# CapAI/ship-sim-gym

Hardware: AMD Instinct MI355X
Metric: env steps/sec (batched ShipEnv) (higher is better)
Workload: dtype f64

## Files before the change

### ship_sim_gym_amd/csrc/shipsim_kernels.hip

```cpp
#include <hip/hip_runtime.h>

#include <cfloat>
#include <cstdint>
#include <type_traits>

#include "shipsim.h"
#include "shipsim_internal.h"

namespace ssg {

__device__ __forceinline__ double *lds_base()
{
    extern __shared__ double s_lds[];
    return s_lds;
}

__device__ __forceinline__ double dmin(double a, double b) { return __builtin_fmin(a, b); }
__device__ __forceinline__ double dmax(double a, double b) { return __builtin_fmax(a, b); }

__device__ __forceinline__ double obs_fma(double a, double b, double c)
{
#ifndef SSG_NO_LIDAR_FMA
    return __builtin_fma(a, b, c);
#else
    return a * b + c;
#endif
}

__device__ __forceinline__ double readlane_f64(double v, int src_lane)
{
    const int lo = __builtin_amdgcn_readlane(__double2loint(v), src_lane);
    const int hi = __builtin_amdgcn_readlane(__double2hiint(v), src_lane);
    return __hiloint2double(hi, lo);
}

__device__ __forceinline__ void set_f64(double &d, double v) { asm volatile("v_mov_b64 %0, %1" : "+v"(d) : "v"(v)); }
__device__ __forceinline__ void set_f64_uniform(double &d, double s) { asm volatile("v_mov_b64 %0, %1" : "+v"(d) : "s"(s)); }
__device__ __forceinline__ void set_f64_zero(double &d) { asm volatile("v_mov_b64 %0, 0" : "+v"(d)); }
__device__ __forceinline__ void set_f64_one(double &d) { asm volatile("v_mov_b64 %0, 1.0" : "+v"(d)); }
__device__ __forceinline__ void set_f64_minus_one(double &d) { asm volatile("v_mov_b64 %0, -1.0" : "+v"(d)); }
template <class T> __device__ __forceinline__ void set_b32(T &d, T v) { static_assert(sizeof(T) == 4, "one register"); asm volatile("v_mov_b32 %0, %1" : "+v"(d) : "v"(v)); }
__device__ __forceinline__ void set_b32_uniform(int &d, int s) { asm volatile("v_mov_b32 %0, %1" : "+v"(d) : "s"(s)); }
template <class T> __device__ __forceinline__ void set_b32_zero(T &d) { static_assert(sizeof(T) == 4, "one register"); asm volatile("v_mov_b32 %0, 0" : "+v"(d)); }

__device__ __attribute__((noinline)) double2 sincos_call(double a)
{
    double2 o;
    sincos_body(a, &o.x, &o.y);
    return o;
}

__device__ __forceinline__ double ld_f64(const double *p, bool fresh)
{
    if (fresh)
        return __longlong_as_double((long long)__hip_atomic_load(reinterpret_cast<const unsigned long long *>(p),
                                                                  __ATOMIC_RELAXED, __HIP_MEMORY_SCOPE_AGENT));
    return *p;
}
__device__ __forceinline__ int ld_i32(const int32_t *p, bool fresh)
{
    if (fresh) return __hip_atomic_load(p, __ATOMIC_RELAXED, __HIP_MEMORY_SCOPE_AGENT);
    return *p;
}
__device__ __forceinline__ unsigned ld_u8(const uint8_t *p, bool fresh)
{
    if (fresh) return __hip_atomic_load(p, __ATOMIC_RELAXED, __HIP_MEMORY_SCOPE_AGENT);
    return *p;
}

template <bool LDS_BANK>
__device__ __forceinline__ double bank_at(const DevCfg &c, int i)
{
    if constexpr (LDS_BANK) return lds_base()[i];
    else return c.bank[i];
}
template <bool LDS_BANK>
__device__ __forceinline__ double2 bank_at2(const DevCfg &c, int i)
{
    if constexpr (LDS_BANK) { double2 r; r.x = lds_base()[i]; r.y = lds_base()[i + 1]; return r; }
    else {
        typedef double double2_a8 __attribute__((ext_vector_type(2), aligned(8)));
        const double2_a8 v = *reinterpret_cast<const double2_a8 *>(c.bank + i);
        double2 r; r.x = v.x; r.y = v.y; return r;
    }
}

template <int THREADS>
__device__ __forceinline__ void stage_bank_lds(const double *__restrict__ bank, int bytes, double &tail_v, int &tail_o)
{
    const int wave = threadIdx.x >> 6, lane = threadIdx.x & 63;
    constexpr int NW = THREADS / 64;
    const int nchunk = bytes >> 10;
    const char *g = reinterpret_cast<const char *>(bank);
    char *l = reinterpret_cast<char *>(lds_base());
    for (int ch = wave; ch < nchunk; ch += NW) {
        __builtin_amdgcn_global_load_lds((const __attribute__((address_space(1))) void *)(g + (size_t)ch * 1024 + lane * 16),
                                         (__attribute__((address_space(3))) void *)(l + ch * 1024), 16, 0, 0);
    }
    const int tail0 = nchunk << 10;
    const int o = tail0 + (int)threadIdx.x * 8;
    tail_o = (o < bytes) ? o : -1;
    tail_v = 0.0;
    if (o < bytes) tail_v = *reinterpret_cast<const double *>(g + o);
    static_assert(THREADS * 8 >= 1024, "tail copy needs one thread per 8 bytes of a 1 KiB chunk");
}

template <bool LDS_BANK, bool DYN>
__device__ __forceinline__ double goal_at(const DevCfg &c, int goff, int g, int comp)
{
    if constexpr (DYN) return c.dyn_f64[(size_t)(DC_GOALS + DC_GOAL_COLS * g + comp) * (size_t)c.n_pad + goff];
    else return bank_at<LDS_BANK>(c, goff + 2 * g + comp);
}

template <bool LDS_BANK, bool DYN>
__device__ __forceinline__ void nearest_goal(const DevCfg &c, int goff, unsigned gm, double x, double y, double &gx,
                                             double &gy, const double *hG = nullptr , int ld = 0)
{
    gx = -1.0;
    gy = -1.0;
    double best = INFINITY;
    int gi = -1;
    if constexpr (!LDS_BANK && !DYN) {
#pragma unroll
        for (int g = 0; g < SSG_MAX_GOALS; ++g) {
            if (g >= c.n_goals) break;
            const double px = hG[(2 * g) * ld], py = hG[(2 * g + 1) * ld];
// ... 36 lines not shown
}

__device__ __forceinline__ int next_map(const DevCfg &c, int map_id, int env)
{
    if (c.map_ring > 0) {
        const int base = env * c.map_ring;
        const int nxt = map_id + 1;
        return (nxt - base >= c.map_ring) ? base : nxt;
    }
    const int nxt = map_id + 1;
    return (nxt >= c.n_maps) ? 0 : nxt;
}

__device__ __forceinline__ void beam_end(double cx, double cy, double ca, double sa, double cphi, double sphi, double dist,
                                         double &ex, double &ey)
{
    const double ux = obs_fma(ca, cphi, -(sa * sphi)), uy = obs_fma(sa, cphi, ca * sphi);
    ex = obs_fma(dist, ux, cx);
    ey = obs_fma(dist, uy, cy);
}

__host__ __device__ __forceinline__ constexpr int nb_lo(int nb) { return (nb + 1) / 2; }
constexpr int kBeamTabBytes = 2 * SSG_MAX_BEAMS * 8;
constexpr int kShipTabBytes = 6 * 8 * 8;
constexpr int kTrafficTabBytes = SSG_N_TRAFFIC * 4 * 8 * 8;
constexpr int kPoseDoubles = 7;
constexpr int kGoalScratchBytes = 64 * SSG_MAX_GOALS * 2 + 64 * 4;
constexpr int kTrafficScratchBytes = 64 * SSG_N_TRAFFIC * 2 + 64 * 4;
__host__ __device__ __forceinline__ constexpr int lds_fixed_bytes(int epw, bool dyn)
{
    return kBeamTabBytes + kShipTabBytes + (dyn ? kTrafficTabBytes : 0) + kPoseDoubles * epw * 8 + (dyn ? 8 : 6) * epw * 4 + 4 * (epw / 64) * 4 +
           (epw / 64) * (kGoalScratchBytes + (dyn ? kTrafficScratchBytes : 0));
}
__host__ __device__ __forceinline__ constexpr int lds_res_bytes(int nb) { return nb * 64 * 8; }
__host__ __device__ __forceinline__ constexpr int lds_queue_bytes(int nb0) { return (2 * nb0 * 64 + 64) * 2; }
__host__ __device__ __forceinline__ constexpr int lds_tile_bytes(int nb)
{
    return 2 * lds_res_bytes(nb) + 2 * lds_queue_bytes(nb_lo(nb));
}

constexpr int kHdrLidar = 10, kHdrGoals = 2 * SSG_MAX_GOALS;
static_assert(SSG_MAP_OFF_COUNTS == 0 && SSG_MAP_OFF_AABB == 2 && SSG_MAP_OFF_GOALS == kHdrLidar && SSG_MAP_OFF_SPAWN_GOAL == kHdrLidar + kHdrGoals,
              "the record's head: counts, boxes, goals, spawn goal");
#ifndef SSG_SIX_ROLE_MAX_EPW
#define SSG_SIX_ROLE_MAX_EPW 128
#endif
__host__ __device__ __forceinline__ constexpr int tile_roles(int epw, bool dyn) { return (epw <= SSG_SIX_ROLE_MAX_EPW && !dyn) ? 6 : 4; }
__host__ __device__ __forceinline__ constexpr int lds_hdr_bytes(int epw, bool lds_bank, bool dyn) { return lds_bank ? 0 : ((tile_roles(epw, dyn) - 2) * kHdrLidar + kHdrGoals) * epw * 8; }

constexpr unsigned long long kLidarMiss = ~0ull;

template <bool LDS_BANK> struct PlaneChunk { static constexpr int n = LDS_BANK ? 4 : 8; };

template <bool EXACT>
__device__ __forceinline__ double seg_mad(double a, double b, double c) { return EXACT ? a * b + c : obs_fma(a, b, c); }

template <bool LDS_BANK, bool EXACT>
__device__ __forceinline__ void lidar_pass(const DevCfg &c, const int n_items, const unsigned short *queue,
                                           unsigned long long *res , const double *beamtab,
                                           const double cx, const double cy, const double ca, const double sa,
                                           const int rec_off, const int lane, const double *hLt = nullptr , const int ld = 0)
{
    for (int base = 0; base < n_items; base += 64) {
        const int idx = base + lane;
        const bool act = idx < n_items;
        const unsigned code = queue[act ? idx : 0];
        const int src = code & 63, bi = (code >> 6) & (SSG_MAX_BEAMS - 1), s = (code >> 10) & 1;
        const double wcx = __shfl(cx, src), wcy = __shfl(cy, src), wca = __shfl(ca, src), wsa = __shfl(sa, src);
        const int woff = __shfl(rec_off, src);
        double ex, ey;
        beam_end(wcx, wcy, wca, wsa, beamtab[bi], beamtab[SSG_MAX_BEAMS + bi], c.lidar_dist, ex, ey);
        int cnt;
        if constexpr (LDS_BANK) cnt = (int)bank_at<LDS_BANK>(c, woff + SSG_MAP_OFF_COUNTS + s);
        else cnt = (int)hLt[s * ld + src];
        const int pb = woff + SSG_MAP_OFF_PLANES + s * (SSG_MAX_HULL * SSG_PLANE_DOUBLES);
        bool outside = false;
        bool out_sure = false, maybe = false;
        constexpr double kSignEps = 1e-9;
        bool ok = false;
        double ptx = ex, pty = ey;
        double bd = -1.0, bden = 1.0, t_hit = 0.0;
        int bj = 0;
        constexpr int kPlaneChunk = PlaneChunk<LDS_BANK>::n;
        for (int j0 = 0; __any(act & (j0 < cnt)); j0 += kPlaneChunk) {
            double pv0x[kPlaneChunk], pv0y[kPlaneChunk], pnx[kPlaneChunk], pny[kPlaneChunk], pv0n[kPlaneChunk];
            double pdtmin[kPlaneChunk], pdtmax[kPlaneChunk];
#pragma unroll
            for (int u = 0; u < kPlaneChunk; ++u) {
                const int j = j0 + u;
                const int q = pb + SSG_PLANE_DOUBLES * ((j < SSG_MAX_HULL) ? j : 0);
                const bool want = LDS_BANK || (act & (j < cnt));
                pv0x[u] = pv0y[u] = pnx[u] = pny[u] = pv0n[u] = 0.0;
                if (EXACT && want) { const double2 vv = bank_at2<LDS_BANK>(c, q + 0); pv0x[u] = vv.x; pv0y[u] = vv.y; }
                if (want) { const double2 nn = bank_at2<LDS_BANK>(c, q + 2); pnx[u] = nn.x; pny[u] = nn.y; }
                if (want) pv0n[u] = bank_at<LDS_BANK>(c, q + 4);
                if (EXACT) {
                    const int jp = (j == 0) ? cnt - 1 : j - 1;
                    const int qp = pb + SSG_PLANE_DOUBLES * ((jp >= 0 && jp < SSG_MAX_HULL) ? jp : 0);
                    const double ux = bank_at<LDS_BANK>(c, qp + 0), uy = bank_at<LDS_BANK>(c, qp + 1);
                    pdtmin[u] = seg_mad<EXACT>(pnx[u], uy, -(pny[u] * ux));
                    pdtmax[u] = seg_mad<EXACT>(pnx[u], pv0y[u], -(pny[u] * pv0x[u]));
                }
            }
#pragma unroll
            for (int u = 0; u < kPlaneChunk; ++u) {
                const int j = j0 + u;
                const bool valid = act & (j < cnt);
                const double nx = pnx[u], ny = pny[u], v0n = pv0n[u];
                const double an = seg_mad<EXACT>(wcx, nx, wcy * ny);
                const double d = an - v0n;
                if (EXACT) {
                    outside = outside | (valid & ((nx * (wcx - pv0x[u]) + ny * (wcy - pv0y[u])) > 0.0));
                } else {
                    out_sure = out_sure | (valid & (d > kSignEps));
                    maybe = maybe | (valid & !(d < -kSignEps));
                }
                const bool front = valid & !(d < 0.0);
                const double bn = seg_mad<EXACT>(ex, nx, ey * ny);
                const double den = dmax(an - bn, DBL_MIN);
                if (EXACT) {
                    const double t = d / den;
                    const double omt = 1.0 - t;
                    const double qx = seg_mad<EXACT>(ex, t, wcx * omt), qy = seg_mad<EXACT>(ey, t, wcy * omt);
                    const double dtv = seg_mad<EXACT>(nx, qy, -(ny * qx));
                    const bool acc = front & !((t < 0.0) | (1.0 < t)) & (pdtmin[u] <= dtv) & (dtv <= pdtmax[u]);
                    ok = ok | acc;
                    ptx = acc ? qx : ptx;
                    pty = acc ? qy : pty;
                } else {
                    const bool better = front & (d <= den) & (d * bden >= bd * den);
#ifdef SSG_NO_MASKED_BEST
                    bd = better ? d : bd;
                    bden = better ? den : bden;
                    bj = better ? j : bj;
#else
                    if (better) { set_f64(bd, d); set_f64(bden, den); set_b32_uniform(bj, j); }
#endif
                }
            }
        }
        if (!EXACT) {
            outside = out_sure;
            const bool need_exact = act & !out_sure & maybe;
            if (__any(need_exact)) {
                bool o = false;
                for (int j = 0; __any(need_exact & (j < cnt)); ++j) {
                    const int qq = pb + SSG_PLANE_DOUBLES * ((j < SSG_MAX_HULL) ? j : 0);
                    const double v0x = bank_at<LDS_BANK>(c, qq + 0), v0y = bank_at<LDS_BANK>(c, qq + 1);
                    const double nx = bank_at<LDS_BANK>(c, qq + 2), ny = bank_at<LDS_BANK>(c, qq + 3);
                    o = o | ((j < cnt) & ((nx * (wcx - v0x) + ny * (wcy - v0y)) > 0.0));
                }
                outside = need_exact ? o : outside;
            }
            const int q = pb + SSG_PLANE_DOUBLES * bj;
            const int jp = (bj == 0) ? cnt - 1 : bj - 1;
            const int qp = pb + SSG_PLANE_DOUBLES * ((jp >= 0 && jp < SSG_MAX_HULL) ? jp : 0);
            double2 nn = bank_at2<LDS_BANK>(c, q + 2), vj = bank_at2<LDS_BANK>(c, q + 0), vp = bank_at2<LDS_BANK>(c, qp + 0);
            if constexpr (!LDS_BANK) asm volatile("" : "+v"(nn.x), "+v"(nn.y), "+v"(vj.x), "+v"(vj.y), "+v"(vp.x), "+v"(vp.y));
            const double nx = nn.x, ny = nn.y;
            const double dtmin = obs_fma(nx, vp.y, -(ny * vp.x));
            const double dtmax = obs_fma(nx, vj.y, -(ny * vj.x));
            const double t = bd / bden;
            const double omt = 1.0 - t;
            ptx = obs_fma(ex, t, wcx * omt);
            pty = obs_fma(ey, t, wcy * omt);
            const double dtv = obs_fma(nx, pty, -(ny * ptx));
            ok = (bd >= 0.0) & (dtmin <= dtv) & (dtv <= dtmax);
            t_hit = t;
        }
        const bool hit = act & (ok | !outside);
        double dist;
        if constexpr (EXACT) {
            const double px = outside ? ptx : ex, py = outside ? pty : ey;
            const double dx = px - wcx, dy = py - wcy;
            dist = sqrt(dx * dx + dy * dy);
        } else {
            dist = outside ? t_hit * c.lidar_dist : c.lidar_dist;
        }
        if (hit) {
            const unsigned long long key = ((unsigned long long)s << 63) | (unsigned long long)__double_as_longlong(dist);
            atomicMin(&res[bi * 64 + src], key);
        }
#ifdef SSG_LIDAR_COUNT
        if (c.dbg) {
            const unsigned long long ma = __ballot(act), mh = __ballot(hit), mo = __ballot(act & !outside);
            if (lane == 0) { atomicAdd(c.dbg + 65536 + 0, (unsigned long long)__popcll(ma)); atomicAdd(c.dbg + 65536 + 1, (unsigned long long)__popcll(mh));
                             atomicAdd(c.dbg + 65536 + 2, 1ull); atomicAdd(c.dbg + 65536 + 3, (unsigned long long)__popcll(mo)); }
        }
#endif
    }
}

template <class T>
__device__ __forceinline__ void st_out(T *p, T v)
{
#ifdef SSG_WT
    __hip_atomic_store(p, v, __ATOMIC_RELAXED, __HIP_MEMORY_SCOPE_AGENT);
#else
    *p = v;
#endif
}

#ifdef SSG_STAMPS
#define SSG_STAMP(k)                                                                              \
    do {                                                                                          \
        __builtin_amdgcn_sched_barrier(0);                                                        \
        unsigned long long t_;                                                                    \
        asm volatile("s_memtime %0\n\ts_waitcnt lgkmcnt(0)" : "=s"(t_)::"memory");               \
        __builtin_amdgcn_sched_barrier(0);                                                        \
        stamp_[k] = t_;                                                                           \
    } while (0)
#define SSG_STAMP_FLUSH(n)                                                                        \
    do {                                                                                          \
        if (c.dbg && lane == 0) {                                                                 \
            unsigned long long *d_ = c.dbg + 16 * (size_t)(blockIdx.x * (NR * EPW / 64) + (threadIdx.x >> 6)); \
            for (int k_ = 0; k_ < 16; ++k_) d_[k_] = stamp_[k_];   \
        }                                                                                         \
    } while (0)
#ifdef SSG_STAMPS_ITER
#define SSG_STAMP_K(i) do { } while (0)
#else
#define SSG_STAMP_K(i) do { if (k == (K >= 2 ? K - 2 : 0)) SSG_STAMP(i); } while (0)
#endif
#else
// ... 10 lines not shown
#define SSG_CLOCK_END()                                                                            \
    do {                                                                                           \
        if (c.dbg && blockIdx.x == 0 && threadIdx.x == 0) {                                        \
            c.dbg[0] = __builtin_amdgcn_s_memtime() - clk_c0_;                                     \
            c.dbg[1] = __builtin_amdgcn_s_memrealtime() - clk_r0_;                                 \
        }                                                                                          \
    } while (0)
#endif

#ifdef SSG_ABLATION
#define SSG_ABL(bit) (c.flags & (1u << (16 + (bit))))
#else
#define SSG_ABL(bit) false
#endif

__device__ __forceinline__ void ship_world(const double *shiptab, double ca, double sa, double x, double y,
                                           double (&swx)[SSG_SHIP_VERTS], double (&swy)[SSG_SHIP_VERTS], double &sbl,
                                           double &sbr, double &sbb, double &sbt)
{
    sbl = INFINITY; sbr = -INFINITY; sbb = INFINITY; sbt = -INFINITY;
#pragma unroll
    for (int i = 0; i < SSG_SHIP_VERTS; ++i) {
        const double hx = shiptab[0 * 8 + i], hy = shiptab[1 * 8 + i];
        swx[i] = ca * hx + (-sa) * hy + x;
        swy[i] = sa * hx + ca * hy + y;
        sbl = dmin(sbl, swx[i]); sbr = dmax(sbr, swx[i]);
        sbb = dmin(sbb, swy[i]); sbt = dmax(sbt, swy[i]);
    }
}

template <int NB, bool LDS_BANK, bool EXACT>
__device__ __forceinline__ void lidar_query(const DevCfg &c, unsigned long long *res, unsigned short *queue,
                                            const double *beamtab, const int b_first, const int b_count, const double cx,
                                            const double cy, const double ca, const double sa, const int rec_off,
                                            const bool live, const int lane, const double *hL = nullptr , const int ld = 0)
{
    constexpr int NB0 = nb_lo(NB);
    constexpr int kTrash = 2 * NB0 * 64;
    int n_items = 0;
    const double eps = 1e-6;
    double al[2], ab[2], ar[2], at[2];
#pragma unroll
    for (int s = 0; s < 2; ++s) {
        double2 lb, rt;
        if constexpr (LDS_BANK) {
            lb = bank_at2<LDS_BANK>(c, rec_off + SSG_MAP_OFF_AABB + 4 * s + 0);
            rt = bank_at2<LDS_BANK>(c, rec_off + SSG_MAP_OFF_AABB + 4 * s + 2);
        } else {
            lb.x = hL[(SSG_MAP_OFF_AABB + 4 * s + 0) * ld]; lb.y = hL[(SSG_MAP_OFF_AABB + 4 * s + 1) * ld];
            rt.x = hL[(SSG_MAP_OFF_AABB + 4 * s + 2) * ld]; rt.y = hL[(SSG_MAP_OFF_AABB + 4 * s + 3) * ld];
        }
        al[s] = lb.x - eps;
        ab[s] = lb.y - eps;
        ar[s] = rt.x + eps;
        at[s] = rt.y + eps;
    }
    (void)ab; (void)at; (void)al; (void)ar;
#ifdef SSG_QUEUE_BEAM_MAJOR
#pragma unroll
    for (int k = 0; k < NB0; ++k) {
        if (k < b_count) {
            const int i = b_first + k;
            res[i * 64 + lane] = kLidarMiss;
            if (!SSG_ABL(1)) {
                double ex, ey;
                beam_end(cx, cy, ca, sa, beamtab[i], beamtab[SSG_MAX_BEAMS + i], c.lidar_dist, ex, ey);
                const double lox = dmin(cx, ex), hix = dmax(cx, ex), loy = dmin(cy, ey), hiy = dmax(cy, ey);
#pragma unroll
                for (int s = 0; s < 2; ++s) {
                    const bool need = live & (lox <= ar[s]) & (al[s] <= hix) & (loy <= at[s]) & (ab[s] <= hiy);
                    const unsigned long long m = __ballot(need);
                    const int pos = n_items + (int)__builtin_amdgcn_mbcnt_hi((unsigned)(m >> 32),
                                                                              __builtin_amdgcn_mbcnt_lo((unsigned)m, 0u));
                    queue[need ? pos : (kTrash + lane)] = (unsigned short)(lane | (k << 6) | (s << 10));
                    n_items += __popcll(m);
                }
            }
        }
    }
#else
    unsigned needmask = 0u;
    bool need[2 * NB0] = {};
    const double lca = c.lidar_dist * ca, lsa = c.lidar_dist * sa;
    const bool org0 = live & (cx <= ar[0]), org1 = live & (al[1] <= cx);
#pragma unroll
    for (int k = 0; k < NB0; ++k) {
        if (k < b_count) {
            const int i = b_first + k;
            res[i * 64 + lane] = kLidarMiss;
            if (!SSG_ABL(1)) {
                const double ex = obs_fma(lca, beamtab[i], obs_fma(-lsa, beamtab[SSG_MAX_BEAMS + i], cx));
                need[2 * k + 0] = org0 | (live & (ex <= ar[0]));
                need[2 * k + 1] = org1 | (live & (al[1] <= ex));
                needmask |= need[2 * k + 0] ? (1u << (2 * k + 0)) : 0u;
                needmask |= need[2 * k + 1] ? (1u << (2 * k + 1)) : 0u;
            }
        }
    }
    {
        const int cnt = __popc(needmask);
        int incl = cnt;
        incl += __builtin_amdgcn_update_dpp(0, incl, 0x111, 0xF, 0xF, false);
        incl += __builtin_amdgcn_update_dpp(0, incl, 0x112, 0xF, 0xF, false);
        incl += __builtin_amdgcn_update_dpp(0, incl, 0x114, 0xF, 0xF, false);
        incl += __builtin_amdgcn_update_dpp(0, incl, 0x118, 0xF, 0xF, false);
        incl += __builtin_amdgcn_update_dpp(0, incl, 0x142, 0xA, 0xF, false);
        incl += __builtin_amdgcn_update_dpp(0, incl, 0x143, 0xC, 0xF, false);
        n_items = __builtin_amdgcn_readlane(incl, 63);
        unsigned nm = needmask;
        asm volatile("" : "+v"(nm));
        char *qp = reinterpret_cast<char *>(queue) + 2 * (incl - cnt);
#pragma unroll
        for (int k = 0; k < NB0; ++k) {
            if (k < b_count) {
#pragma unroll
                for (int s = 0; s < 2; ++s) {
                    if (need[2 * k + s]) *reinterpret_cast<unsigned short *>(qp) = (unsigned short)(lane | (k << 6) | (s << 10));
                    qp += 2u * ((nm >> (2 * k + s)) & 1u);
                }
            }
        }
        (void)kTrash;
    }
#endif
    if (!SSG_ABL(3))
        lidar_pass<LDS_BANK, EXACT>(c, n_items, queue, res + b_first * 64, beamtab + b_first, cx, cy, ca, sa, rec_off, lane,
                                    hL ? hL - lane : nullptr, ld);
}

template <int NB>
struct ObsTile {
    static constexpr int FF = 6 + NB;
    static constexpr int CS = (NB >= 2) ? 73 : 64;
    static constexpr int CP = (NB * 64) / CS;
    static_assert(CP >= 1 && CP * CS * 8 <= lds_res_bytes(NB), "observation chunk does not fit the lidar result buffer");
    static constexpr bool kOnTheFly = (CP & (CP - 1)) == 0;
    int lds_at[kOnTheFly ? 1 : CP];
    int row[kOnTheFly ? 1 : CP], col[kOnTheFly ? 1 : CP];
    __device__ __forceinline__ void init(int lane)
    {
        if constexpr (!kOnTheFly) {
#pragma unroll
            for (int jj = 0; jj < CP; ++jj) {
                const int t = lane + 64 * jj;
                row[jj] = t / CP;
                col[jj] = t - row[jj] * CP;
                lds_at[jj] = col[jj] * CS + row[jj];
            }
        }
    }
    __device__ __forceinline__ int row_of(int jj, int lane) const { if constexpr (kOnTheFly) return (lane + 64 * jj) / CP; else return row[jj]; }
    __device__ __forceinline__ int col_of(int jj, int lane) const { if constexpr (kOnTheFly) return (lane + 64 * jj) % CP; else return col[jj]; }
    __device__ __forceinline__ int lds_of(int jj, int lane) const { if constexpr (kOnTheFly) return col_of(jj, lane) * CS + row_of(jj, lane); else return lds_at[jj]; }
};

template <int NB, bool H2, int P_BEGIN, int P_END, class Val>
__device__ __forceinline__ void write_obs_tile(const ObsTile<NB> &ot, double *colbuf, const Val &val ,
                                               double *__restrict__ obase, const int rows_live, const int lane)
{
    constexpr int FF = 6 + NB;
    constexpr int DH = H2 ? 2 * FF : FF;
    constexpr int CS = ObsTile<NB>::CS, CP = ObsTile<NB>::CP;
    int lds_at[CP], gl_at[CP];
    unsigned okmask = 0;
    int ln_ = lane;
    asm volatile("" : "+v"(ln_));
#pragma unroll
    for (int jj = 0; jj < CP; ++jj) {
        lds_at[jj] = ot.lds_of(jj, ln_);
        gl_at[jj] = ot.row_of(jj, ln_) * DH + ot.col_of(jj, ln_);
        okmask |= (ot.row_of(jj, ln_) < rows_live) ? (1u << jj) : 0u;
        if constexpr (!ObsTile<NB>::kOnTheFly) asm volatile("" : "+v"(lds_at[jj]), "+v"(gl_at[jj]));
    }
    asm volatile("" : "+v"(okmask));
#pragma unroll
    for (int pi = P_BEGIN; pi < P_END; ++pi) {
        const int p0 = pi * CP;
        if (p0 >= DH) break;
        const int cpp = (DH - p0 < CP) ? (DH - p0) : CP;
#pragma unroll
        for (int cc = 0; cc < CP; ++cc) {
            if (cc < cpp) colbuf[cc * CS + lane] = val(p0 + cc);
        }
        if (cpp == CP) {
#pragma unroll
            for (int jj = 0; jj < CP; ++jj) {
                const double v = colbuf[lds_at[jj]];
                if ((okmask >> jj) & 1u) st_out(&obase[(unsigned)(gl_at[jj] + p0)], v);
            }
        } else {
            int ln = lane;
            asm volatile("" : "+v"(ln));
#pragma unroll
            for (int jj = 0; jj < CP; ++jj) {
                if (jj < cpp) {
                    const int t = ln + 64 * jj;
                    const int r = t / cpp, cc = t - r * cpp;
                    const double v = colbuf[cc * CS + r];
                    if (r < rows_live) st_out(&obase[(unsigned)(r * DH + p0 + cc)], v);
                }
            }
        }
        __builtin_amdgcn_sched_barrier(0);
    }
}

template <int NB, bool H2, int C_BEGIN, int C_END, class Val>
__device__ __forceinline__ void write_obs_pairs(double *buf , const Val &val ,
                                                double *__restrict__ obase, const int rows_live, const int lane)
{
    constexpr int FF = 6 + NB;
    constexpr int DH = H2 ? 2 * FF : FF;
    static_assert(C_BEGIN % 2 == 0 && C_END % 2 == 0 && DH % 2 == 0 && NB >= 8, "pairs of columns; 64 x 8 doubles of buffer");
    int ln = lane;
    asm volatile("" : "+v"(ln));
    char *const bufc = reinterpret_cast<char *>(buf);
    char *const outc = reinterpret_cast<char *>(obase);
    const unsigned uln = (unsigned)ln;
    const unsigned wrow = uln << 6, wsw16 = (uln << 2) & 48u;
    const unsigned r4 = uln >> 2, q4 = uln & 3u;
    const unsigned l4 = (r4 << 6) + (((q4 ^ (uln >> 4)) & 3u) << 4), g4 = (r4 * DH + 2u * q4) * 8u;
    const unsigned r2 = uln >> 1, q2 = uln & 1u;
    const unsigned l2 = (r2 << 6) + ((q2 ^ ((uln >> 3) & 3u)) << 4), g2 = (r2 * DH + 2u * q2) * 8u;
#pragma unroll
    for (int c0 = C_BEGIN; c0 < C_END; c0 += 8) {
        constexpr int kMax = 4;
        const int np = ((C_END - c0) / 2 < kMax) ? (C_END - c0) / 2 : kMax;
#pragma unroll
        for (int q = 0; q < kMax; ++q)
            if (q < np) *reinterpret_cast<double2 *>(bufc + (wrow + (wsw16 ^ (16u * q)))) = make_double2(val(c0 + 2 * q), val(c0 + 2 * q + 1));
#pragma unroll
        for (int jj = 0; jj < kMax; ++jj) {
            if (jj < np) {
                if (np == 4 || np == 2 || np == 1) {
                    const int rstep = 64 / np;
                    const unsigned r0 = (np == 4) ? r4 : (np == 2) ? r2 : uln;
                    const unsigned lat = (np == 4) ? l4 : (np == 2) ? l2 : wrow + wsw16;
                    const unsigned gat = (np == 4) ? g4 : (np == 2) ? g2 : uln * (DH * 8u);
                    const double2 v = *reinterpret_cast<const double2 *>(bufc + jj * rstep * 64 + lat);
                    if ((int)r0 < rows_live - jj * rstep)
                        *reinterpret_cast<double2 *>(outc + (size_t)((jj * rstep * DH + c0) * 8) + gat) = v;
                } else {
                    const int pidx = ln + 64 * jj;
                    const int r = pidx / 3;
                    const int q = pidx - r * np;
                    const double2 v = *reinterpret_cast<const double2 *>(buf + r * 8 + 2 * (q ^ ((r >> 2) & 3)));
                    if (r < rows_live) *reinterpret_cast<double2 *>(&obase[(unsigned)(r * DH + c0 + 2 * q)]) = v;
                }
            }
        }
        __builtin_amdgcn_sched_barrier(0);
    }
}

template <bool LDS_BANK>
__device__ __forceinline__ bool bank_narrowphase(const DevCfg &c, const double *shiptab, const double x, const double y,
                                                 const double ca, const double sa, const int rec_off, const bool live,
                                                 const int lane, const int only ,
                                                 const double *hL = nullptr ,
                                                 const int ld = 0)
{
    const int wq = lane / 5, wi = lane - 5 * wq;
    const double w_hx = shiptab[0 * 8 + wi], w_hy = shiptab[1 * 8 + wi];
    const double w_nx = shiptab[2 * 8 + wi], w_ny = shiptab[3 * 8 + wi];
    double swx[SSG_SHIP_VERTS], swy[SSG_SHIP_VERTS], sbl, sbr, sbb, sbt;
    ship_world(shiptab, ca, sa, x, y, swx, swy, sbl, sbr, sbb, sbt);
    bool colliding = false;
    unsigned nearbits = 0;
    int cnts = 0;
#pragma unroll
    for (int s = 0; s < 2; ++s) {
        double al, ab, ar, at, cn;
        if constexpr (LDS_BANK) {
            const double2 lb = bank_at2<LDS_BANK>(c, rec_off + SSG_MAP_OFF_AABB + 4 * s + 0);
            const double2 rt = bank_at2<LDS_BANK>(c, rec_off + SSG_MAP_OFF_AABB + 4 * s + 2);
            al = lb.x; ab = lb.y; ar = rt.x; at = rt.y;
            cn = bank_at<LDS_BANK>(c, rec_off + SSG_MAP_OFF_COUNTS + s);
        } else {
            al = hL[(SSG_MAP_OFF_AABB + 4 * s + 0) * ld]; ab = hL[(SSG_MAP_OFF_AABB + 4 * s + 1) * ld];
            ar = hL[(SSG_MAP_OFF_AABB + 4 * s + 2) * ld]; at = hL[(SSG_MAP_OFF_AABB + 4 * s + 3) * ld];
            cn = hL[(SSG_MAP_OFF_COUNTS + s) * ld];
        }
        const bool near = live & !SSG_ABL(4) & ((only < 0) | (only == s)) & (sbl <= ar) & (al <= sbr);
        (void)ab; (void)at; (void)sbb; (void)sbt;
        nearbits |= near ? (1u << s) : 0u;
        cnts |= ((int)cn) << (8 * s);
    }
#pragma unroll
    for (int s = 0; s < 2; ++s) {
        const bool near_s = (nearbits >> s) & 1u;
        if (!__any(near_s)) continue;
        const int cnt = (cnts >> (8 * s)) & 0xFF;
        bool sep = false;
        if constexpr (LDS_BANK) {
            for (int j = 0; __any(near_s & !sep & (j < cnt)); ++j) {
                if (near_s & !sep & (j < cnt)) {
                    const int q = rec_off + SSG_MAP_OFF_PLANES + s * (SSG_MAX_HULL * SSG_PLANE_DOUBLES) + SSG_PLANE_DOUBLES * j;
                    const double2 nn = bank_at2<LDS_BANK>(c, q + 2);
                    const double nx = nn.x, ny = nn.y;
                    const double v0n = bank_at<LDS_BANK>(c, q + 4);
                    bool allfront = true;
#pragma unroll
                    for (int i = 0; i < SSG_SHIP_VERTS; ++i) allfront = allfront & ((nx * swx[i] + ny * swy[i]) > v0n);
                    sep = allfront;
                }
            }
        } else {
            constexpr int kNpChunk = 4;
            for (int j0 = 0; __any(near_s & !sep & (j0 < cnt)); j0 += kNpChunk) {
                if (near_s & !sep & (j0 < cnt)) {
                    double nx[kNpChunk], ny[kNpChunk], v0n[kNpChunk];
#pragma unroll
                    for (int u = 0; u < kNpChunk; ++u) {
                        const int j = (j0 + u < SSG_MAX_HULL) ? j0 + u : 0;
                        const int q = rec_off + SSG_MAP_OFF_PLANES + s * (SSG_MAX_HULL * SSG_PLANE_DOUBLES) + SSG_PLANE_DOUBLES * j;
                        const double2 nn = bank_at2<LDS_BANK>(c, q + 2);
                        nx[u] = nn.x; ny[u] = nn.y;
                        v0n[u] = bank_at<LDS_BANK>(c, q + 4);
                    }
#pragma unroll
                    for (int u = 0; u < kNpChunk; ++u) {
                        bool allfront = j0 + u < cnt;
#pragma unroll
                        for (int i = 0; i < SSG_SHIP_VERTS; ++i) allfront = allfront & ((nx[u] * swx[i] + ny[u] * swy[i]) > v0n[u]);
                        sep = sep | allfront;
                    }
                }
            }
        }
        nearbits = sep ? (nearbits & ~(1u << s)) : nearbits;
    }
    unsigned long long todo = __ballot(nearbits != 0u);
// ... 353 lines not shown
                if (rs | (key != kLidarMiss)) st_out(&colLid[(size_t)i * np + el_], rs ? -1.0 : hitd);
            }
        }
        SSG_STAMP(10);
        SSG_STAMP_FLUSH(3);
        SSG_CLOCK_END();
        return;
    }

    if constexpr (NR == 6) {
        if (role >= 4) {
            const int h = role - 4;
            int map0 = colMap[el_];
            if constexpr (!LDS_BANK) load_hdr_lidar(map0 * SSG_MAP_STRIDE);
            asm volatile("" : "+v"(map0));
            flush_tables();
            if (LDS_BANK) __builtin_amdgcn_s_waitcnt(0);
            __syncthreads();
            SSG_STAMP(9);
            for (int k = 0; k < K; ++k) {
                wait_pose(k);
                SSG_STAMP_K(0);
                const double nca = pose[2 * EPW + tl], nsa = pose[3 * EPW + tl];
                const double npx = pose[0 * EPW + tl], npy = pose[1 * EPW + tl];
                const int nmap = posem[tl];
                ack_pose();
                reinterpret_cast<unsigned short *>(gres)[2 * ((k & 1) * EPW + tl) + h] =
                        bank_narrowphase<LDS_BANK>(c, shiptab, npx, npy, nca, nsa, nmap * SSG_MAP_STRIDE, live, lane, h, hL, EPW) ? 1 : 0;
                SSG_STAMP_K(1);
                tile_barrier(k);
                SSG_STAMP_K(2);
                if constexpr (!LDS_BANK) {
                    if (k + 1 < K) {
                        const bool rs = auto_reset & ((gres[(k & 1) * EPW + tl] | (gdone[(k & 1) * EPW + tl] & 1u)) != 0u);
                        if (rs) load_hdr_lidar(next_map(c, nmap, el_) * SSG_MAP_STRIDE);
                    }
                }
            }
            SSG_STAMP(10);
            SSG_STAMP_FLUSH(5);
            return;
        }
    }

    const int wq = lane / 5, wi = lane - 5 * wq;

    if (role == 2) {
        constexpr int F = 6 + NB;
        double pv[F];
        double ogp[DYN ? 2 * SSG_MAX_GOALS : 1];
        unsigned gm_pre = 0u;
        {
            const int el = el_;
            const double x0 = colX[el], y0 = colY[el], a0 = colA[el];
            const int rud0 = colRud[el], map0 = colMap[el];
            const unsigned gm0 = c.mask[el];
#pragma unroll
            for (int i = 0; i < NB; ++i) pv[6 + i] = colLid[(size_t)i * np + el];
            pv[0] = x0; pv[1] = y0; pv[2] = (double)rud0; pv[3] = a0;
            if constexpr (DYN) {
                pv[4] = c.dyn_f64[(size_t)(DC_PREV_GOAL + 0) * np + el];
                pv[5] = c.dyn_f64[(size_t)(DC_PREV_GOAL + 1) * np + el];
            }
#pragma unroll
            for (int i = 0; i < 4; ++i) asm volatile("" : "+v"(pv[i]));
#pragma unroll
            for (int i = 0; i < NB; ++i) asm volatile("" : "+v"(pv[6 + i]));
            if constexpr (DYN) asm volatile("" : "+v"(pv[4]), "+v"(pv[5]));
            int map0_ = map0; unsigned gm0_ = gm0;
            asm volatile("" : "+v"(map0_), "+v"(gm0_));
            gm_pre = gm0_;
            flush_tables();
            if (LDS_BANK) __builtin_amdgcn_s_waitcnt(0);
            __syncthreads();
            SSG_STAMP(9);
            if constexpr (!DYN)
                nearest_goal<LDS_BANK, false>(c, map0_ * SSG_MAP_STRIDE + SSG_MAP_OFF_GOALS, gm0_, pv[0], pv[1], pv[4], pv[5], hG, EPW);
        }
        const bool hist2 = c.history >= 2;
        ObsTile<NB> ot;
        ot.init(lane);
        constexpr int kObsPasses = (2 * F + ObsTile<NB>::CP - 1) / ObsTile<NB>::CP;
        constexpr bool kPairs = (NB >= 8) && (NB % 2 == 0);
        constexpr bool kSplitOk = kPairs || (F % ObsTile<NB>::CP) == 0;
        const bool split_last = kSplitOk && hist2 && c.history == 2 && !SSG_ABL(7);
        for (int k = 0; k < K; ++k) {
            const bool early = split_last && (k == K - 1);
            if constexpr (kSplitOk) {
                if (early) {
                    int tw = __builtin_amdgcn_readfirstlane(tl >> 6);
                    int te0 = blockIdx.x * EPW + 64 * tw;
                    asm volatile("" : "+s"(tw), "+s"(te0));
                    double *colbuf = reinterpret_cast<double *>(scratch0 + tw * lds_tile_bytes(NB) + ((k + 1) & 1) * lds_res_bytes(NB));
                    double *__restrict__ ob = obs + ((size_t)te0 + (size_t)k * (size_t)traj) * (size_t)(2 * F);
                    if constexpr (kPairs)
                        write_obs_pairs<NB, true, 0, F>(colbuf, [&](int j) -> double { return pv[(j < F) ? j : 0]; }, ob, min(64, c.n_envs - te0), lane);
                    else
                        write_obs_tile<NB, true, 0, F / ObsTile<NB>::CP>(ot, colbuf, [&](int j) -> double { return pv[(j < F) ? j : 0]; }, ob,
                                                                        min(64, c.n_envs - te0), lane);
                }
            }
            if constexpr (DYN) {
#pragma unroll
                for (int g = 0; g < SSG_MAX_GOALS; ++g) {
                    const bool listed = g < c.n_goals;
                    ogp[2 * g] = listed ? goal_at<LDS_BANK, DYN>(c, el_, g, 0) : 0.0;
                    ogp[2 * g + 1] = listed ? goal_at<LDS_BANK, DYN>(c, el_, g, 1) : 0.0;
                }
            }
            wait_pose(k);
            if constexpr (DYN) {
#pragma unroll
                for (int g = 0; g < 2 * SSG_MAX_GOALS; ++g) asm volatile("" : "+v"(ogp[g]));
            }
            SSG_STAMP_K(0);
            const double x = pose[0 * EPW + tl], y = pose[1 * EPW + tl];
            const double ang = pose[6 * EPW + tl];
            const int rudder = poser[tl];
            const int map_id = posem[tl];
            ack_pose();
            const int rec_off = map_id * SSG_MAP_STRIDE;
            SSG_STAMP_K(1);
#ifdef SSG_NO_SPEC
            const bool spec = false;
#else
            const bool spec = kSplitOk && NR == 4 && early && !SSG_ABL(7);
#endif
            double sp_gx = 0.0, sp_gy = 0.0;
            if (kSplitOk && spec) {
                wait_queries();
                const unsigned listed_pre = gm_pre & ((1u << c.n_goals) - 1u);
                if constexpr (DYN) nearest_goal_regs(c.n_goals, listed_pre, x, y, ogp, sp_gx, sp_gy);
                else nearest_goal<LDS_BANK, false>(c, rec_off + SSG_MAP_OFF_GOALS, listed_pre, x, y, sp_gx, sp_gy, hG, EPW);
                double sv[F];
                sv[0] = x; sv[1] = y; sv[2] = (double)rudder; sv[3] = ang; sv[4] = sp_gx; sv[5] = sp_gy;
                int tw = __builtin_amdgcn_readfirstlane(tl >> 6);
                int te0 = blockIdx.x * EPW + 64 * tw;
                asm volatile("" : "+s"(tw), "+s"(te0));
                const unsigned long long *rk = reinterpret_cast<const unsigned long long *>(scratch0 + tw * lds_tile_bytes(NB) + (k & 1) * lds_res_bytes(NB));
#pragma unroll
                for (int i = 0; i < NB; ++i) {
                    const unsigned long long key = rk[i * 64 + lane];
                    const double hitd = __longlong_as_double((long long)(key & 0x7FFFFFFFFFFFFFFFull));
                    sv[6 + i] = (key == kLidarMiss) ? pv[6 + i] : hitd;
                }
                double *colbuf = reinterpret_cast<double *>(scratch0 + tw * lds_tile_bytes(NB) + ((k + 1) & 1) * lds_res_bytes(NB));
                double *__restrict__ ob = obs + ((size_t)te0 + (size_t)k * (size_t)traj) * (size_t)(2 * F);
                if constexpr (kPairs)
                    write_obs_pairs<NB, true, F, 2 * F>(colbuf, [&](int j) -> double { return sv[(j < F) ? 0 : j - F]; }, ob, min(64, c.n_envs - te0), lane);
                else
                    write_obs_tile<NB, true, kSplitOk ? F / ObsTile<NB>::CP : 0, kObsPasses>(ot, colbuf, [&](int j) -> double {
                        return sv[(j < F) ? 0 : j - F]; }, ob, min(64, c.n_envs - te0), lane);
            }
            tile_barrier(k);
            SSG_STAMP_K(2);

            const unsigned gd = gdone[(k & 1) * EPW + tl];
            const bool colliding = (gres[(k & 1) * EPW + tl] != 0u) | (DYN && traffic_hit(k) != 0u);
            const bool do_reset = auto_reset & (colliding | ((gd & 1u) != 0u));
            if (live && k < K - 1) {
                const bool goal_reached = (gd & 4u) != 0u;
                double rew = goal_reached ? 1.0 : ((gd & 8u) ? -1.0 : -0.01);
                if ((c.flags & SSG_FLAG_FIX_COLLISION_REWARD) && (colliding & !goal_reached)) rew = -1.0;
                const size_t eo = (size_t)el_ + (size_t)k * (size_t)traj;
                st_out(&reward_out[eo], rew);
                st_out(&done_out[eo], (uint8_t)((colliding | ((gd & 1u) != 0u)) ? 1 : 0));
                if (flags_out) {
                    unsigned ev = 0;
                    if (colliding) ev |= SSG_EV_COLLIDING;
                    if (goal_reached) ev |= SSG_EV_GOAL_REACHED;
                    if (gd & 8u) ev |= SSG_EV_OUT_OF_BOUNDS;
                    if (gd & 16u) ev |= SSG_EV_MAX_STEPS;
                    if (gd & 32u) ev |= SSG_EV_NO_GOALS_LEFT;
                    st_out(&flags_out[eo], (uint8_t)ev);
                }
            }
            SSG_STAMP_K(4);
            double nf_gx = sp_gx, nf_gy = sp_gy;
            if (!spec || __any((gd >> 8) != (gm_pre & ((1u << c.n_goals) - 1u)))) {
                if constexpr (DYN) nearest_goal_regs(c.n_goals, gd >> 8, x, y, ogp, nf_gx, nf_gy);
                else if (!SSG_ABL(0)) nearest_goal<LDS_BANK, false>(c, rec_off + SSG_MAP_OFF_GOALS, gd >> 8, x, y, nf_gx, nf_gy, hG, EPW);
            }
            SSG_STAMP_K(5);
            int tile_w = __builtin_amdgcn_readfirstlane(tl >> 6);
            int tile_e0 = blockIdx.x * EPW + 64 * tile_w;
            asm volatile("" : "+s"(tile_w), "+s"(tile_e0));
            char *res_k = scratch0 + tile_w * lds_tile_bytes(NB) + (k & 1) * lds_res_bytes(NB);
            const int map_new = do_reset ? next_map(c, map_id, el_) : map_id;
            double rs_gx = 0.0, rs_gy = 0.0;
            if (LDS_BANK || do_reset) {
                const double2 sg = bank_at2<LDS_BANK>(c, map_new * SSG_MAP_STRIDE + SSG_MAP_OFF_SPAWN_GOAL);
                rs_gx = sg.x; rs_gy = sg.y;
            }
            double nv[F];
            nv[0] = x; nv[1] = y; nv[2] = (double)rudder; nv[3] = ang; nv[4] = nf_gx; nv[5] = nf_gy;
            {
                const unsigned long long *rk = reinterpret_cast<const unsigned long long *>(res_k);
#pragma unroll
                for (int i = 0; i < NB; ++i) {
                    const unsigned long long key = rk[i * 64 + lane];
                    const double hitd = __longlong_as_double((long long)(key & 0x7FFFFFFFFFFFFFFFull));
                    nv[6 + i] = (key == kLidarMiss) ? pv[6 + i] : hitd;
                }
            }
            if (c.term_obs != nullptr && traj == 0 && do_reset && live) {
                double *trow = c.term_obs + (size_t)el_ * (size_t)(F * c.history) + (hist2 ? F : 0);
                if (hist2) {
#pragma unroll
                    for (int j = 0; j < F; ++j) st_out(&trow[j - F], pv[j]);
                }
                st_out(&trow[0], x); st_out(&trow[1], y); st_out(&trow[2], (double)rudder); st_out(&trow[3], ang);
                st_out(&trow[4], nf_gx); st_out(&trow[5], nf_gy);
#pragma unroll
                for (int i = 0; i < NB; ++i) st_out(&trow[6 + i], nv[6 + i]);
            }
            const bool hist_whole = hist2 && !(kSplitOk && (spec || early));
            if (do_reset) {
                set_f64_uniform(nv[0], c.spawn_x); set_f64_uniform(nv[1], c.spawn_y);
                set_f64_zero(nv[2]); set_f64_zero(nv[3]);
                set_f64(nv[4], rs_gx); set_f64(nv[5], rs_gy);
#pragma unroll
                for (int i = 0; i < NB; ++i) set_f64_minus_one(nv[6 + i]);
                if (hist_whole) {
#pragma unroll
                    for (int j = 0; j < F; ++j) set_f64_minus_one(pv[j]);
                }
            }
            SSG_STAMP_K(6);
            {
                double *__restrict__ obase = obs + ((size_t)tile_e0 + (size_t)k * (size_t)traj) * (size_t)(F * c.history);
                const int rows_live = min(64, c.n_envs - tile_e0);
                if (!SSG_ABL(7)) {
                    double *colbuf = reinterpret_cast<double *>((K == 1) ? res_k + lds_res_bytes(NB) : res_k);
                    if (kSplitOk && spec) {
                        const bool goal_moved = !do_reset & ((nf_gx != sp_gx) | (nf_gy != sp_gy));
                        if (__any(do_reset | goal_moved)) {
                            __builtin_amdgcn_s_waitcnt(0x0F70);
                            if (lane < rows_live) {
                                if (do_reset) {
#pragma unroll
                                    for (int j = 0; j < F; ++j) st_out(&obase[(unsigned)(lane * 2 * F + j)], -1.0);
#pragma unroll
                                    for (int j = 0; j < F; ++j) st_out(&obase[(unsigned)(lane * 2 * F + F + j)], nv[j]);
                                } else if (goal_moved) {
                                    st_out(&obase[(unsigned)(lane * 2 * F + F + 4)], nv[4]);
                                    st_out(&obase[(unsigned)(lane * 2 * F + F + 5)], nv[5]);
                                }
                            }
                        }
                    } else if (kSplitOk && early) {
                        if (__any(do_reset)) {
                            __builtin_amdgcn_s_waitcnt(0x0F70);
                            if (do_reset && lane < rows_live) {
#pragma unroll
                                for (int j = 0; j < F; ++j) st_out(&obase[(unsigned)(lane * 2 * F + j)], -1.0);
                            }
                        }
                        if constexpr (kPairs)
                            write_obs_pairs<NB, true, F, 2 * F>(colbuf, [&](int j) -> double { return nv[(j < F) ? 0 : j - F]; }, obase, rows_live, lane);
                        else
                            write_obs_tile<NB, true, kSplitOk ? F / ObsTile<NB>::CP : 0, kObsPasses>(ot, colbuf, [&](int j) -> double {
                                return nv[(j < F) ? 0 : j - F]; }, obase, rows_live, lane);
                    } else if (hist2) {
                        if constexpr (kPairs)
                            write_obs_pairs<NB, true, 0, 2 * F>(colbuf, [&](int j) -> double {
                                return (j < F) ? pv[(j < F) ? j : 0] : nv[(j < F) ? 0 : j - F]; }, obase, rows_live, lane);
                        else
                            write_obs_tile<NB, true, 0, kObsPasses>(ot, colbuf, [&](int j) -> double {
                                return (j < F) ? pv[(j < F) ? j : 0] : nv[(j < F) ? 0 : j - F]; },
                                obase, rows_live, lane);
                    } else {
                        if constexpr (kPairs)
                            write_obs_pairs<NB, false, 0, F>(colbuf, [&](int j) -> double { return nv[(j < F) ? j : 0]; }, obase, rows_live, lane);
                        else
                            write_obs_tile<NB, false, 0, kObsPasses>(ot, colbuf, [&](int j) -> double { return nv[(j < F) ? j : 0]; }, obase, rows_live, lane);
                    }
                }
            }
            SSG_STAMP_K(7);
            if constexpr (DYN) {
                if (live) {
                    c.dyn_f64[(size_t)(DC_PREV_GOAL + 0) * np + el_] = nv[4];
                    c.dyn_f64[(size_t)(DC_PREV_GOAL + 1) * np + el_] = nv[5];
                }
            }
#pragma unroll
            for (int i = 0; i < F; ++i) pv[i] = nv[i];
            gm_pre = do_reset ? ((1u << c.n_goals) - 1u) : (gd >> 8);
            if (k == K - 1 && K > 1 && live && !SSG_ABL(9)) {
                int el = el_;
                asm volatile("" : "+v"(el));
#pragma unroll
                for (int i = 0; i < NB; ++i) st_out(&colLid[(size_t)i * np + el], pv[6 + i]);
            }
            SSG_STAMP_K(3);
        }
        SSG_STAMP(10);
        SSG_STAMP_FLUSH(4);
        return;
    }

    double x, y, vx, vy, ang, w, cum;
    unsigned gm;
    int map_id, rudder, steps, episodes;
    {
        const int el = el_;
        x = colX[el]; y = colY[el]; vx = colVX[el]; vy = colVY[el]; ang = colA[el]; w = colW[el]; cum = colCum[el];
        gm = c.mask[el];
        map_id = colMap[el];
        rudder = colRud[el];
        steps = colStep[el];
        episodes = c.i32cols[(size_t)ICOL_EPISODE * np + el];
    }
    if constexpr (!LDS_BANK && !DYN) load_hdr_goals(map_id * SSG_MAP_STRIDE);
    int act_next = actions_kn[el_];
    double gpre[DYN ? 2 * SSG_MAX_GOALS : 1];
    unsigned dflag = 0;
    unsigned long long dlive = 0ull;
    auto ask_goals = [&]() {
#pragma unroll
        for (int g = 0; g < SSG_MAX_GOALS; ++g) {
            const bool listed = g < c.n_goals;
            gpre[2 * g] = listed ? goal_at<LDS_BANK, DYN>(c, el_, g, 0) : 0.0;
            gpre[2 * g + 1] = listed ? goal_at<LDS_BANK, DYN>(c, el_, g, 1) : 0.0;
        }
        dflag = c.dyn_flag[el_];
        dlive = c.dyn_live[el_];
    };
    auto have_goals = [&]() {
#pragma unroll
        for (int g = 0; g < 2 * SSG_MAX_GOALS; ++g) asm volatile("" : "+v"(gpre[g]));
        asm volatile("" : "+v"(dflag), "+v"(dlive));
    };
    asm volatile("" : "+v"(x), "+v"(y), "+v"(vx), "+v"(vy), "+v"(ang), "+v"(w), "+v"(cum));
    asm volatile("" : "+v"(gm), "+v"(map_id), "+v"(rudder), "+v"(steps), "+v"(episodes), "+v"(act_next));
    flush_tables();
    if (LDS_BANK) __builtin_amdgcn_s_waitcnt(0);
    __syncthreads();
    SSG_STAMP(9);
    if constexpr (DYN) ask_goals();
    const double w_hx = shiptab[0 * 8 + wi], w_hy = shiptab[1 * 8 + wi];
    const double w_nx = shiptab[2 * 8 + wi], w_ny = shiptab[3 * 8 + wi];
#ifdef SSG_PRIO
    __builtin_amdgcn_s_setprio(SSG_PRIO);
#endif

    bool q_need = false;
    long long st_ret = 0;
    int st_len = 0, st_eps = 0, st_goals = 0;
    unsigned q_bucket = 0, q_arrival = 0;
    for (int k = 0; k < K; ++k) {
#ifdef SSG_STAMPS_ITER
    if (k < 8) SSG_STAMP(k);
    if (k == K - 1) SSG_STAMP(11);
    if (k == 12) SSG_STAMP(12);
    if (k == 16) SSG_STAMP(13);
// ... 503 lines not shown
```

Before: 13.93 billion.

## Use inline-asm cmpx masking in lidar plane loop and batch obs pair stores

Replaces the per-plane best-hit selection in the non-exact lidar path with hand-written GCN assembly. It uses v_cmpx to narrow exec, accumulates the outside/maybe masks in scalar registers, and skips the updates when no lanes remain. It also folds the liveness predicate into NaN sentinels for the lidar bank-need tests. Separately, obs pair writes now gather all LDS reads into registers before issuing the global stores, with an unguarded fast path when the full tile is live. The aim is to cut VALU mask work and interleaved LDS/global waits, at the cost of fragile inline asm and higher register pressure.

```diff
diff --git a/ship_sim_gym_amd/csrc/shipsim_kernels.hip b/ship_sim_gym_amd/csrc/shipsim_kernels.hip
--- a/ship_sim_gym_amd/csrc/shipsim_kernels.hip
+++ b/ship_sim_gym_amd/csrc/shipsim_kernels.hip
@@ -42,6 +42,31 @@
 template <class T> __device__ __forceinline__ void set_b32(T &d, T v) { static_assert(sizeof(T) == 4, "one register"); asm volatile("v_mov_b32 %0, %1" : "+v"(d) : "v"(v)); }
 __device__ __forceinline__ void set_b32_uniform(int &d, int s) { asm volatile("v_mov_b32 %0, %1" : "+v"(d) : "s"(s)); }
 template <class T> __device__ __forceinline__ void set_b32_zero(T &d) { static_assert(sizeof(T) == 4, "one register"); asm volatile("v_mov_b32 %0, 0" : "+v"(d)); }
+
+__device__ __forceinline__ void plane_best_lanes(unsigned long long valid, double d, double den, double p, double q, double eps, int j ,
+                                                 double &bd, double &bden, int &bj, unsigned long long &out_sure, unsigned long long &maybe)
+{
+    unsigned long long sv;
+    asm volatile("s_and_saveexec_b64 %[sv], %[valid]\n\t"
+                 "v_cmp_lt_f64 vcc, %[eps], %[d]\n\t"
+                 "s_or_b64 %[os], %[os], vcc\n\t"
+                 "v_cmp_nlt_f64_e64 vcc, %[d], -%[eps]\n\t"
+                 "s_or_b64 %[mb], %[mb], vcc\n\t"
+                 "v_cmpx_nlt_f64_e64 vcc, %[d], 0\n\t"
+                 "v_cmpx_le_f64 vcc, %[d], %[den]\n\t"
+                 "v_cmpx_ge_f64 vcc, %[p], %[q]\n\t"
+                 "s_cbranch_execz 1f\n\t"
+                 "v_mov_b64 %[bd], %[d]\n\t"
+                 "v_mov_b64 %[bden], %[den]\n\t"
+                 "v_mov_b32 %[bj], %[j]\n"
+                 "1:\n\t"
+                 "s_mov_b64 exec, %[sv]"
+                 : [sv] "=&s"(sv), [os] "+s"(out_sure), [mb] "+s"(maybe), [bd] "+v"(bd), [bden] "+v"(bden), [bj] "+v"(bj)
+                 : [valid] "s"(valid), [d] "v"(d), [den] "v"(den), [p] "v"(p), [q] "v"(q), [eps] "s"(eps), [j] "s"(j)
+                 : "vcc");
+    asm volatile("" : "+s"(out_sure));
+    asm volatile("" : "+s"(maybe));
+}
 
 __device__ __attribute__((noinline)) double2 sincos_call(double a)
 {
@@ -244,7 +269,14 @@
         double bd = -1.0, bden = 1.0, t_hit = 0.0;
         int bj = 0;
         constexpr int kPlaneChunk = PlaneChunk<LDS_BANK>::n;
-        for (int j0 = 0; __any(act & (j0 < cnt)); j0 += kPlaneChunk) {
+#ifdef SSG_NO_CMPX_LIDAR
+        constexpr bool kCmpx = false;
+#else
+        constexpr bool kCmpx = !EXACT && LDS_BANK;
+#endif
+        const int cnt_a = act ? cnt : 0;
+        unsigned long long os_m = 0ull, mb_m = 0ull;
+        for (int j0 = 0; kCmpx ? __any(j0 < cnt_a) : __any(act & (j0 < cnt)); j0 += kPlaneChunk) {
             double pv0x[kPlaneChunk], pv0y[kPlaneChunk], pnx[kPlaneChunk], pny[kPlaneChunk], pv0n[kPlaneChunk];
             double pdtmin[kPlaneChunk], pdtmax[kPlaneChunk];
 #pragma unroll
@@ -267,10 +299,16 @@
 #pragma unroll
             for (int u = 0; u < kPlaneChunk; ++u) {
                 const int j = j0 + u;
-                const bool valid = act & (j < cnt);
                 const double nx = pnx[u], ny = pny[u], v0n = pv0n[u];
                 const double an = seg_mad<EXACT>(wcx, nx, wcy * ny);
                 const double d = an - v0n;
+                if constexpr (kCmpx) {
+                    const double bn = seg_mad<EXACT>(ex, nx, ey * ny);
+                    const double den = dmax(an - bn, DBL_MIN);
+                    plane_best_lanes(__ballot(j < cnt_a), d, den, d * bden, bd * den, kSignEps, j, bd, bden, bj, os_m, mb_m);
+                    continue;
+                }
+                const bool valid = act & (j < cnt);
                 if (EXACT) {
                     outside = outside | (valid & ((nx * (wcx - pv0x[u]) + ny * (wcy - pv0y[u])) > 0.0));
                 } else {
@@ -302,6 +340,10 @@
             }
         }
         if (!EXACT) {
+            if constexpr (kCmpx) {
+                out_sure = __builtin_amdgcn_inverse_ballot_w64(os_m);
+                maybe = __builtin_amdgcn_inverse_ballot_w64(mb_m);
+            }
             outside = out_sure;
             const bool need_exact = act & !out_sure & maybe;
             if (__any(need_exact)) {
@@ -478,7 +520,19 @@
     unsigned needmask = 0u;
     bool need[2 * NB0] = {};
     const double lca = c.lidar_dist * ca, lsa = c.lidar_dist * sa;
-    const bool org0 = live & (cx <= ar[0]), org1 = live & (al[1] <= cx);
+#ifdef SSG_NO_CMPX_LIDAR
+    constexpr bool kFoldLive = false;
+#else
+    constexpr bool kFoldLive = LDS_BANK;
+#endif
+    double ar0 = ar[0], al1 = al[1];
+    if constexpr (kFoldLive) {
+        ar0 = live ? ar0 : __builtin_nan("");
+        al1 = live ? al1 : __builtin_nan("");
+        asm volatile("" : "+v"(ar0), "+v"(al1));
+    }
+    const bool live_ = kFoldLive | live;
+    const bool org0 = live_ & (cx <= ar0), org1 = live_ & (al1 <= cx);
 #pragma unroll
     for (int k = 0; k < NB0; ++k) {
         if (k < b_count) {
@@ -486,8 +540,8 @@
             res[i * 64 + lane] = kLidarMiss;
             if (!SSG_ABL(1)) {
                 const double ex = obs_fma(lca, beamtab[i], obs_fma(-lsa, beamtab[SSG_MAX_BEAMS + i], cx));
-                need[2 * k + 0] = org0 | (live & (ex <= ar[0]));
-                need[2 * k + 1] = org1 | (live & (al[1] <= ex));
+                need[2 * k + 0] = org0 | (live_ & (ex <= ar0));
+                need[2 * k + 1] = org1 | (live_ & (al1 <= ex));
                 needmask |= need[2 * k + 0] ? (1u << (2 * k + 0)) : 0u;
                 needmask |= need[2 * k + 1] ? (1u << (2 * k + 1)) : 0u;
             }
@@ -601,7 +655,7 @@
     }
 }
 
-template <int NB, bool H2, int C_BEGIN, int C_END, class Val>
+template <int NB, bool H2, int C_BEGIN, int C_END, bool BATCH, class Val>
 __device__ __forceinline__ void write_obs_pairs(double *buf , const Val &val ,
                                                 double *__restrict__ obase, const int rows_live, const int lane)
 {
@@ -625,6 +679,52 @@
 #pragma unroll
         for (int q = 0; q < kMax; ++q)
             if (q < np) *reinterpret_cast<double2 *>(bufc + (wrow + (wsw16 ^ (16u * q)))) = make_double2(val(c0 + 2 * q), val(c0 + 2 * q + 1));
+        if constexpr (BATCH) {
+            typedef double d2v __attribute__((ext_vector_type(2)));
+            d2v pc[kMax];
+            unsigned pg[kMax];
+            int pr[kMax];
+#pragma unroll
+            for (int jj = 0; jj < kMax; ++jj) {
+                if (jj < np) {
+                    if (np == 4 || np == 2 || np == 1) {
+                        const int rstep = 64 / np;
+                        const unsigned lat = (np == 4) ? l4 : (np == 2) ? l2 : wrow + wsw16;
+                        pc[jj] = *reinterpret_cast<const d2v *>(bufc + jj * rstep * 64 + lat);
+                    } else {
+                        const int pidx = ln + 64 * jj;
+                        const int r = pidx / 3;
+                        const int q = pidx - r * np;
+                        pc[jj] = *reinterpret_cast<const d2v *>(buf + r * 8 + 2 * (q ^ ((r >> 2) & 3)));
+                        pr[jj] = r;
+                        pg[jj] = (unsigned)(r * DH + c0 + 2 * q) * 8u;
+                    }
+                }
+            }
+            if (np == 4) asm volatile("" : "+v"(pc[0]), "+v"(pc[1]), "+v"(pc[2]), "+v"(pc[3]));
+            else if (np == 3) asm volatile("" : "+v"(pc[0]), "+v"(pc[1]), "+v"(pc[2]));
+            else if (np == 2) asm volatile("" : "+v"(pc[0]), "+v"(pc[1]));
+            else asm volatile("" : "+v"(pc[0]));
+            auto put = [&](auto guarded_) {
+                constexpr bool kGuarded = decltype(guarded_)::value;
+#pragma unroll
+                for (int jj = 0; jj < kMax; ++jj) {
+                    if (jj < np) {
+                        if (np == 4 || np == 2 || np == 1) {
+                            const int rstep = 64 / np;
+                            const unsigned r0 = (np == 4) ? r4 : (np == 2) ? r2 : uln;
+                            const unsigned gat = (np == 4) ? g4 : (np == 2) ? g2 : uln * (DH * 8u);
+                            if (!kGuarded || (int)r0 < rows_live - jj * rstep)
+                                *reinterpret_cast<d2v *>(outc + (size_t)((jj * rstep * DH + c0) * 8) + gat) = pc[jj];
+                        } else {
+                            if (!kGuarded || pr[jj] < rows_live) *reinterpret_cast<d2v *>(outc + pg[jj]) = pc[jj];
+                        }
+                    }
+                }
+            };
+            if (rows_live >= 64) put(std::false_type{});
+            else put(std::true_type{});
+        } else {
 #pragma unroll
         for (int jj = 0; jj < kMax; ++jj) {
             if (jj < np) {
@@ -644,6 +744,7 @@
                     if (r < rows_live) *reinterpret_cast<double2 *>(&obase[(unsigned)(r * DH + c0 + 2 * q)]) = v;
                 }
             }
+        }
         }
         __builtin_amdgcn_sched_barrier(0);
     }
@@ -1163,6 +1264,11 @@
         ot.init(lane);
         constexpr int kObsPasses = (2 * F + ObsTile<NB>::CP - 1) / ObsTile<NB>::CP;
         constexpr bool kPairs = (NB >= 8) && (NB % 2 == 0);
+#ifdef SSG_NO_ROW_BATCH
+        constexpr bool kRowBatch = false;
+#else
+        constexpr bool kRowBatch = !DYN;
+#endif
         constexpr bool kSplitOk = kPairs || (F % ObsTile<NB>::CP) == 0;
         const bool split_last = kSplitOk && hist2 && c.history == 2 && !SSG_ABL(7);
         for (int k = 0; k < K; ++k) {
@@ -1175,7 +1281,7 @@
                     double *colbuf = reinterpret_cast<double *>(scratch0 + tw * lds_tile_bytes(NB) + ((k + 1) & 1) * lds_res_bytes(NB));
                     double *__restrict__ ob = obs + ((size_t)te0 + (size_t)k * (size_t)traj) * (size_t)(2 * F);
                     if constexpr (kPairs)
-                        write_obs_pairs<NB, true, 0, F>(colbuf, [&](int j) -> double { return pv[(j < F) ? j : 0]; }, ob, min(64, c.n_envs - te0), lane);
+                        write_obs_pairs<NB, true, 0, F, kRowBatch>(colbuf, [&](int j) -> double { return pv[(j < F) ? j : 0]; }, ob, min(64, c.n_envs - te0), lane);
                     else
                         write_obs_tile<NB, true, 0, F / ObsTile<NB>::CP>(ot, colbuf, [&](int j) -> double { return pv[(j < F) ? j : 0]; }, ob,
                                                                         min(64, c.n_envs - te0), lane);
@@ -1228,7 +1334,7 @@
                 double *colbuf = reinterpret_cast<double *>(scratch0 + tw * lds_tile_bytes(NB) + ((k + 1) & 1) * lds_res_bytes(NB));
                 double *__restrict__ ob = obs + ((size_t)te0 + (size_t)k * (size_t)traj) * (size_t)(2 * F);
                 if constexpr (kPairs)
-                    write_obs_pairs<NB, true, F, 2 * F>(colbuf, [&](int j) -> double { return sv[(j < F) ? 0 : j - F]; }, ob, min(64, c.n_envs - te0), lane);
+                    write_obs_pairs<NB, true, F, 2 * F, kRowBatch>(colbuf, [&](int j) -> double { return sv[(j < F) ? 0 : j - F]; }, ob, min(64, c.n_envs - te0), lane);
                 else
                     write_obs_tile<NB, true, kSplitOk ? F / ObsTile<NB>::CP : 0, kObsPasses>(ot, colbuf, [&](int j) -> double {
                         return sv[(j < F) ? 0 : j - F]; }, ob, min(64, c.n_envs - te0), lane);
@@ -1338,13 +1444,13 @@
                             }
                         }
                         if constexpr (kPairs)
-                            write_obs_pairs<NB, true, F, 2 * F>(colbuf, [&](int j) -> double { return nv[(j < F) ? 0 : j - F]; }, obase, rows_live, lane);
+                            write_obs_pairs<NB, true, F, 2 * F, kRowBatch>(colbuf, [&](int j) -> double { return nv[(j < F) ? 0 : j - F]; }, obase, rows_live, lane);
                         else
                             write_obs_tile<NB, true, kSplitOk ? F / ObsTile<NB>::CP : 0, kObsPasses>(ot, colbuf, [&](int j) -> double {
                                 return nv[(j < F) ? 0 : j - F]; }, obase, rows_live, lane);
                     } else if (hist2) {
                         if constexpr (kPairs)
-                            write_obs_pairs<NB, true, 0, 2 * F>(colbuf, [&](int j) -> double {
+                            write_obs_pairs<NB, true, 0, 2 * F, kRowBatch>(colbuf, [&](int j) -> double {
                                 return (j < F) ? pv[(j < F) ? j : 0] : nv[(j < F) ? 0 : j - F]; }, obase, rows_live, lane);
                         else
                             write_obs_tile<NB, true, 0, kObsPasses>(ot, colbuf, [&](int j) -> double {
@@ -1352,7 +1458,7 @@
                                 obase, rows_live, lane);
                     } else {
                         if constexpr (kPairs)
-                            write_obs_pairs<NB, false, 0, F>(colbuf, [&](int j) -> double { return nv[(j < F) ? j : 0]; }, obase, rows_live, lane);
+                            write_obs_pairs<NB, false, 0, F, kRowBatch>(colbuf, [&](int j) -> double { return nv[(j < F) ? j : 0]; }, obase, rows_live, lane);
                         else
                             write_obs_tile<NB, false, 0, kObsPasses>(ot, colbuf, [&](int j) -> double { return nv[(j < F) ? j : 0]; }, obase, rows_live, lane);
                     }
```

Result: no change. 13.98 billion (median of 6 runs) (+0.3%).
